# parlance/ctcdecode

Hardware: AMD Instinct MI355X
Metric: utterances/sec at B=256 T=1000 V=29 beam=100 (higher is better)
Workload: dtype f32; 1 GPU; BASELINE.json configs[1]: CTC prefix beam search, no LM, log-softmax of N(0,1) logits; HBM-resident tensors (input in HBM, the four result tensors left in HBM: `e2e`, with --full, is the host-to-host call); utterances_per_gpu=256, frames=1000, vocab=29, beam_width=100, cutoff_top_n=29, global_batch=256, ranks=1, devices_visible=1, parallelism=single GPU, threads_per_workgroup=default

## Files before the change

ctcdecode_amd/csrc/beam_core.h:

```cpp
#pragma once
#include <stddef.h>
#include <stdint.h>

#include "exact_math.h"
#include "exact_math_f64.h"
#include "lm_tables.h"
#include "stl_emul.h"
#if defined(CTC_ASSUME_CHECKED)
#include <cstdio>
#include <cstdlib>
#endif

#define CTC_RARE(x) __builtin_expect(!!(x), 0)
#if !defined(CTC_SPEC_UP)
#define CTC_SPEC_UP 1.5f
#endif
#if !defined(CTC_SPEC_DN)
#define CTC_SPEC_DN 0.7f
#endif
#if !defined(CTC_SPEC_OVER_SHIFT)
#define CTC_SPEC_OVER_SHIFT 2
#endif
#define CTC_USUAL(x) __builtin_expect(!!(x), 1)

// ... 189 lines not shown
  w.rev_lpc = carve_ptr<float>(deep ? q : p, K);
  w.cch = carve_ptr<int>(p, (size_t)d.Vc_max);
  w.clpbuf = carve_ptr<float>(p, 2 * (size_t)d.Vc_max); w.clp = w.clpbuf;
  w.rank_of = carve_ptr<int16_t>(p, d.use_rank_table ? (size_t)d.V : 0);
  w.skey = carve_ptr<uint32_t>(deep ? q : p, S);
  w.surv = carve_ptr<int>(p, 3 * K + 4);
  const size_t lcap = (d.K <= kSmallK && d.Vc_max <= kMidVc) ? (size_t)kHotCap + 64 : (size_t)kListCap + 4;
  w.bins = carve_ptr<int>(p, kBins + kBins / 16 + 4); w.list = carve_ptr<uint32_t>(p, lcap);
  w.lslot = carve_ptr<int>(p, lcap);
  w.hotge = carve_ptr<int>(p, lcap > (size_t)kListCap + 4 ? (size_t)kHotCap : 0);
#if defined(CTC_EXP_LCP_TABLE)
  w.lcpst = carve_ptr<int>(p, (lcap > (size_t)kListCap + 4 && !d.lm) ? (size_t)7 * kSmallK : 0);
#else
  w.lcpst = nullptr;
#endif
  w.bitmap = carve_ptr<uint32_t>(huge ? q : p, 2 * ((S + 63) / 64 + 17));
  w.wpre = huge ? carve_ptr<uint32_t>(q, (S + 63) / 64 + 2) : reinterpret_cast<uint32_t *>(w.bins);
  w.fin = carve_ptr<int>(BIG ? q : p, d.lm ? 2 * K : K);
  w.apos = carve_ptr<int>(BIG ? q : p, K);
  w.sstack = carve_ptr<int>(p, 3 * (2 * 32 + 2));
  w.vars = carve_ptr<int>(p, VAR_COUNT);
  w.sinfo = carve_ptr<uint32_t>(p, BIG ? K : S);
  w.pos = carve_ptr<uint32_t>(BIG ? q : p, K + 2);
  char *&rr = (BIG || FARREP) ? q : p;
  w.ek = carve_ptr<uint64_t>(rr, huge ? 2 * S : S); w.lr = carve_ptr<uint16_t>(rr, (2 * S + 2) * (huge ? 2 : 1));
  w.stage_skey = deep ? 0 : 1;
  if (far_bytes) *far_bytes = (size_t)(q - far);
  return (size_t)(p - base);
}

struct StreamState {
  int *hdr;
  int *arrays;
  int finish;
};
enum { SH_FRAMES = 0, SH_N, SH_POOL, SH_WLOG, SH_MAXKEY, SH_DANGER, SH_MINKEY,
       SH_SP_PRED, SH_SP_GAP, SH_SP_MARGIN,
       SH_WORDS = 12 };
constexpr int kStateArrays = 14;
constexpr int kStateArraysLm = kStateArrays + kBeamArraysLm;
CTC_HD int state_arrays(int lm) { return lm ? kStateArraysLm : kStateArrays; }

struct StepIn {
  int t;
  int Vc;
  int blank_rank;
  int identity;
  float blank_prob;
};


CTC_HD int div_p2(int v, int d) { return v >> __builtin_ctz((unsigned)d); }
CTC_HD int ceil_div_p2(int v, int d) { return div_p2(v + d - 1, d); }

CTC_HD double ctc_log_f64(double v) {
  return ctcmath::log_f64(v, ctcmath::tables64());
}

CTC_HD int ceil_log2_u32(uint32_t v) {
  return v <= 1u ? 0 : 32 - __builtin_clz(v - 1u);
}
CTC_HD int ceil_log2_u64(uint64_t v) {
  return v <= 1 ? 0 : 64 - __builtin_clzll(v - 1);
}

struct OutRefs {
  int32_t *tok, *ts;
  float *score;
  int32_t *len;
  int32_t *n_results;
  int K, T_stride;
  int32_t *c_hdr, *c_ent;
  uint32_t *c_rag;
  unsigned *c_count;
  unsigned c_cap;
  int32_t *m_hdr, *m_ent, *m_done;
  uint32_t *m_rag;
  unsigned m_cap;
};
enum : int { ST_COMPACT_OVERFLOW = 3, ST_INPUT_TIMEOUT = 4,
             ST_NEED_HOST = 5,
             ST_CB_DANGER = 6 };

struct SlotCtx {
  const Beam *pb;
  int n, Vnb, brank;
  uint64_t vmagic;
};

template <class X>
struct FullSyncView {
  X &x;
  CTC_HD int tid() const { return x.tid(); }
  CTC_HD int nt() const { return x.nt(); }
  CTC_HD void sync() { x.sync_full(); }
  CTC_HD int uni(int v) const { return x.uni(v); }
  CTC_HD void block_scan_u32(uint32_t mine, uint32_t *base_out, uint32_t *total_out) { x.block_scan_u32(mine, base_out, total_out); }
  CTC_HD int lanes() const { return x.lanes(); }
  CTC_HD auto ballot(bool p) const { return x.ballot(p); }
  template <class M> CTC_HD int count(M m) const { return x.count(m); }
  template <class M> CTC_HD int count_below(M m) const { return x.count_below(m); }
  CTC_HD uint32_t first_lane(uint32_t v) const { return x.first_lane(v); }
};

#if defined(CTC_ASSUME_CHECKED)
#define CTC_ASSUME(c) do { if (!(c)) { std::fprintf(stderr, "beam_core.h:%d: assumption violated: %s\n", __LINE__, #c); std::abort(); } } while (0)
#elif defined(__clang__)
#define CTC_ASSUME(c) __builtin_assume(c)
#else
#define CTC_ASSUME(c) do { if (!(c)) __builtin_unreachable(); } while (0)
#endif

template <class X, bool IDENT, int SMALLV = 0, bool LM = false, bool LAZY = false, bool FARREP = LAZY, bool HUGE = false, bool WORDLM = false, bool CB = false>
struct Decoder {
  using EO = EkOps<HUGE>;
  using Ek = typename EO::E;
  using LrT = typename EO::Pos;
  static constexpr int kClsK = SMALLV == 2 ? kMidK : kSmallK, kClsVc = SMALLV == 2 ? kMidVc : kSmallV, kClsSlots = kClsK * (2 + kClsVc);
  CTC_HD Ek *ekp() const { return reinterpret_cast<Ek *>(w.ek); }
  CTC_HD LrT *lrp() const { return reinterpret_cast<LrT *>(w.lr); }
  X &x;
  Work &w;
  const Dims d;
  const int blank;
  PoolNode *pool;
  int *pool_up;
  int *pool_thi;
  bool long_t = false;
  const int pool_cap;
  const uint64_t *tbl;
  const ctclm::LmView *lm;

  CTC_HD Decoder(X &x_, Work &w_, const Dims &d_, int blank_, PoolNode *pool_, int *pool_up_, int pool_cap_, const uint64_t *tbl_,
                 const ctclm::LmView *lm_ = nullptr)
      : x(x_), w(w_), d(d_), blank(blank_), pool(pool_), pool_up(pool_up_), pool_thi(pool_up_ + pool_cap_), pool_cap(pool_cap_), tbl(tbl_), lm(lm_) {
    if (LM) {
      const ctclm::DictNode root = lm->dict[0];
      root_lo = (int)root.mask_lo; root_hi = (int)root.mask_hi; root_fc = (int)root.first_child;
      lm_char_v = lm->char_based != 0; lm_wide_v = lm->dict_wide != 0; lm_space = lm->space_id;
      lm_alpha = lm->alpha; lm_beta = lm->beta;
      lm_dict = lm->dict;
    }
  }
  CTC_HD int node_tstep(const PoolNode &pn, int id) const { return (int)(pn.cht >> 16) | (CTC_RARE(long_t) ? pool_thi[id] << 16 : 0); }
  CTC_HD void set_node_time(int id, int ch, int tstep, float lpc) const {
    pool[id].lpc = lpc;
    pool[id].cht = PoolNode::pack(ch, tstep);
    if (CTC_RARE(long_t)) pool_thi[id] = tstep >> 16;
  }

  CTC_HD float lse(float a, float b) const { return ctcmath::lse(a, b, tbl); }

  static constexpr bool kRankEpoch = SMALLV == 2 && !IDENT && X::kRankEpoch;
  CTC_HD static int16_t rank_tag(int t, int r) { return (int16_t)(uint16_t)((((uint32_t)t & 1023u) << 6) | (uint32_t)r); }
  static constexpr bool kTailZero = IDENT && SMALLV && !LAZY && X::kZeroKeyTail;
  CTC_HD void zero_key_tail(int from) {
    if (!kTailZero) return;
    for (int i = from + x.tid(); i < kClsSlots; i += x.nt()) w.skey[i] = 0u;
  }

  static constexpr bool kSpec = SMALLV && (!LM || (X::kSpecLm && !CB)) && !LAZY && X::kSpecSelect;
#if defined(CTC_EXP_HOT_PRELIST)
  static constexpr bool kHotPre = LAZY && !LM && !SMALLV && !HUGE;
#else
  static constexpr bool kHotPre = false;
#endif
  struct HotPre { uint32_t thr; int cap; uint32_t *key; int *slot; };
  uint32_t st_gap = 0;
  uint32_t hot_anchor = 0;
  static constexpr bool kA1Overlap = kSpec && X::kA1Overlap;
// ... 1569 lines not shown
            } else {
              logp = child_logp(w.anc[j], c, lp);
              o_lpc = w.rev_lpc[j];
            }
            if (LM && lm_scores(c)) logp = lm_apply(logp, lm_window(b, child ? j : w.anc[j], c));
            o_b = CTC_NEG_MAX; o_nb = logp; o_sc = logp;
          }
          nb.bprev[k] = o_b; nb.nbprev[k] = o_nb; nb.score[k] = o_sc; nb.lpc[k] = o_lpc;
        }
        if (r_lm) lm_emit(b, (self || child) ? j : w.anc[j], self ? -1 : c, nb, k);
        if (r_prob) {
          const uint32_t ks = keys_in_ord ? (uint32_t)ord[k] : w.skey[s];
          kloc = ks > kloc ? ks : kloc;
          kmin = ks < kmin ? ks : kmin;
        }
      }
    }
    if (x.uni((int)r_prob_any)) {
      x.wave_max_to(&pv[P_NMAXKEY], kloc);
      if (LM) x.wave_min_to(&pv[P_NMINKEY], kmin);
    }
    if (CTC_RARE(last || exact || (N <= K && x.uni(w.vars[VAR_DANGER]) != 0))) {
      int *fin = fin_nxt();
      for (int q = tid; q < n_new; q += nt) {
        const int r = exact ? rk[q] : q;
        fin[q] = r;
        w.apos[r] = q;
      }
    } else if (lm_cb) {
      const int *fc = fin_cur();
      int *fn = fin_nxt();
      for (int q = tid; q < d.K; q += nt) fn[q] = fc[q];
    }
    if (!IDENT && !kRankEpoch) {
      x.sync();
      for (int r = tid; r < Vc; r += nt) w.rank_of[w.cch[r]] = -1;
    }
    if (stage && tid < d.V) w.clpbuf[((in.t + 1) & 1) * d.Vc_max + tid] = stage_val;
    if ((kSpec || kHotPre) && stage) x.row_max_store(&w.vars[VAR_ROWMAX], stage_val, d.V);
    x.mark(7);
    x.sync_full();
    x.mark(9);
    if (LM && CTC_RARE(lm_cb) && x.uni(w.vars[VAR_LMMISS]) != 0) return ST_NEED_HOST;
    if (kTailZero && LM) {
      const int S_next = n_new * (2 + Vnb);
      if (CTC_RARE(S_next < S))
        for (int i = S_next + tid; i < S; i += nt) w.skey[i] = 0u;
    }
    {
      if (!kSpec) {
        int wl = 32;
        st_gap = 0;
        if (N > K) {
          const uint32_t gap = st_maxkey > tau ? st_maxkey - tau : 0;
          wl = (gap ? 32 - __builtin_clz(gap) : 0) + 1;
          wl = wl < 10 ? 10 : (wl > 32 ? 32 : wl);
          st_gap = kHotPre ? (hot_anchor > tau ? hot_anchor - tau : 0u) : gap;
        }
        st_wlog = wl;
        st_maxkey = (uint32_t)x.uni(pv[P_NMAXKEY]);
      }
      if (LM) st_minkey = (uint32_t)x.uni(pv[P_NMINKEY]);
      st_n = n_new;
      st_pool = pool_count + n_new;
    }
    x.tick();
    x.dump(in.t, n_new, nb.node, nb.dep, nb.lcp, nb.score);
    x.mark(8);
    st_par ^= 1;
    return ST_OK;
  }

  template <class T, class C>
  CTC_HD void sort_like_std(T *v, int n, C before) {
    const int tid = x.tid(), nt = x.nt();
    constexpr int kTaskCap = (kBins + kBins / 16) / 6;
    if (n <= 16 || n / 17 + 1 > kTaskCap) {
      if (tid == 0) stlemu::sort(v, 0, n, before, w.sstack);
      x.sync();
      return;
    }
    stlemu::sort_parallel(x, v, n, before, w.bins, w.bins + 3 * kTaskCap, w.surv, w.vars + VAR_TAU);
  }

  CTC_HD int finish(bool had_steps, int max_depth, const OutRefs *outs, int item) {
    const OutRefs o = *x.fresh(outs);
    const int T_stride = o.T_stride;
    const size_t ko = (size_t)o.K * (size_t)o.T_stride;
    int32_t *out_tok = o.tok + (size_t)item * ko, *out_ts = o.ts + (size_t)item * ko;
    float *out_score = o.score + (size_t)item * o.K;
    int32_t *out_len = o.len + (size_t)item * o.K;
    int32_t *n_results = o.n_results ? o.n_results + item : nullptr;
    select_beams();
    const Beam &b = w.cur;
    const int tid = x.tid(), nt = x.nt();
    const int n = st_n;
    if (SMALLV) { CTC_ASSUME(n >= 1 && n <= kClsK); CTC_ASSUME(d.K <= kClsK); }
    const int nres = n < d.K ? n : d.K;
    if (!had_steps)
      for (int k = tid; k < nres; k += nt) fin_cur()[k] = k;
    x.sync();
    float *ext = w.sc_new;
    float *approx = w.b_new;
    {
      const float *sc = b.score;
      const int *ch = b.ch;
      uint64_t *pk = sort_scratch();
      if (LM) {
        for (int a = tid; a < n; a += nt) {
          if (CTC_RARE(lm_cb) && b.dfc[a] == kLmPending) continue;
          const bool partial = !lm_char_() && b.dep[a] > 0 && ch[a] != lm_space;
          const bool word_here = partial && lm_allows(b, a, lm_space);
          const double wcond = word_here ? mk_f64(b.spc_lo[a], b.spc_hi[a]) : ctclm::kOovScore;
          float e = sc[a];
          if (partial) {
            float score = 0.0f;
            score = (float)(wcond * lm_alpha);
            score = (float)((double)score + lm_beta);
            e += score;
          }
          ext[a] = e;
          double total = mk_f64(b.acc_lo[a], b.acc_hi[a]);
          uint32_t st = (uint32_t)b.lmst[a];
          int cl = b.lmcl[a];
          if (b.dep[a] == 0) {
            total += lm_cond_(&st, &cl, lm->w_bos);
          } else if (partial) {
            total += wcond;
            if (word_here) { st = (uint32_t)b.spst[a]; cl = b.spcl[a]; }
            else {
              st = (lm_cb && lm->clean0 == 0) ? lm->s0 : 0u;
              cl = 0;
            }
          }
          total += lm_cond_(&st, &cl, lm->w_eos);
          double ap = (double)e;
          ap = ap - (double)(size_t)b.dep[a] * lm_beta;
          ap -= total * lm_alpha;
          approx[a] = (float)ap;
        }
        x.sync();
        if (CTC_RARE(lm_cb) && x.uni(w.vars[VAR_LMMISS]) != 0) return ST_NEED_HOST;
      }
      for (int p = tid; p < nres; p += nt) {
        const int a = fin_cur()[p];
        pk[p] = (key48(ord_f32(LM ? ext[a] : sc[a]), mk_info(ch[a], 0, 0)) << 16) | (uint64_t)a;
      }
      x.sync();
      auto before = [](uint64_t a, uint64_t c) { return (a >> 16) > (c >> 16); };
      sort_like_std(pk, nres, before);
      if (LM) {
        for (int p = tid; p < nres; p += nt) {
          const int a = (int)(pk[p] & 0xFFFFu);
          pk[p] = (key48(ord_f32(sc[a]), mk_info(ch[a], 0, 0)) << 16) | (uint64_t)a;
        }
        x.sync();
      }
      sort_like_std(pk, nres, before);
      for (int p = tid; p < nres; p += nt) fin_cur()[p] = (int)(pk[p] & 0xFFFFu);
    }
    if (tid == 0 && n_results) *n_results = nres;
    x.sync();
    for (int p = tid; p < nres; p += nt) {
      const int j = fin_cur()[p];
      out_score[p] = LM ? -approx[j] : -b.score[j];
      out_len[p] = b.dep[j];
    }
    int *row_of = w.pinr, *owner = w.e;
    for (int p = tid; p < nres; p += nt) row_of[fin_cur()[p]] = p;
    for (int j = tid; j < nres; j += nt) {
      int o = j - 1;
      const int l = b.lcp[j];
      while (o >= 0 && b.lcp[o] >= l) --o;
      owner[j] = o;
    }
    x.sync();
    x.mark(4);
    const bool compact = o.c_hdr != nullptr;
    unsigned cbase = 0;
    uint32_t ctotal = 0;
    if (compact) {
      for (int j = tid; j < nres; j += nt) {
        const int lo = b.lcp[j] > 0 ? b.lcp[j] : 0;
        w.pos[j] = (uint32_t)(b.dep[j] > lo ? b.dep[j] - lo : 0);
      }
      if (tid == 0) w.pos[nres] = 0;
      x.sync();
      const uint32_t total = x.scan_excl(w.pos, nres + 1);
      if (tid == 0) w.vars[VAR_CUT] = (int)x.global_add(o.c_count, total);
      x.sync();
      cbase = (unsigned)x.uni(w.vars[VAR_CUT]);
      ctotal = total;
      const bool fits = cbase + total <= o.c_cap && cbase + total >= cbase;
      if (tid == 0) {
        int32_t *h = o.c_hdr + (size_t)item * 4;
        h[0] = fits ? nres : 0; h[1] = fits ? (int32_t)total : 0; h[2] = (int32_t)cbase; h[3] = 0;
        if (!fits) w.vars[VAR_STATUS] = ST_COMPACT_OVERFLOW;
      }
      if (!fits) return ST_COMPACT_OVERFLOW;
      for (int j = tid; j < nres; j += nt) {
        int32_t *e = o.c_ent + ((size_t)item * o.K + j) * 4;
        e[0] = row_of[j]; e[1] = b.lcp[j] > 0 ? b.lcp[j] : 0; e[2] = b.dep[j]; e[3] = (int32_t)(cbase + w.pos[j]);
      }
    }
    const int maxseg = max_depth / kExpress + 1;
    for (int idx = tid; idx < nres * maxseg; idx += nt) {
      const int i = idx / nres, j = idx - i * nres;
      const int dj = b.dep[j];
      const int lo = b.lcp[j] > 0 ? b.lcp[j] : 0;
      const int base = ((dj - 1) / kExpress) * kExpress;
      if (dj <= 0 || i > base / kExpress) continue;
      int dd = i == 0 ? dj : base - (i - 1) * kExpress;
      int stop = i == 0 ? base : dd - kExpress;
      if (dd <= lo) continue;
      stop = stop < lo ? lo : stop;
      int xn;
      if (i == 0) {
        xn = b.node[j];
      } else {
        xn = b.up[j];
        for (int h = 1; h < i; ++h) xn = pool_up[xn];
      }
      if (compact) {
        uint32_t *seg = o.c_rag + (size_t)cbase + w.pos[j] - lo;
        while (dd > stop) {
          const PoolNode pn = pool[xn];
          seg[dd - 1] = pn.cht;
          xn = pn.parent;
          --dd;
        }
        continue;
      }
      const size_t row = (size_t)row_of[j] * T_stride;
      int32_t *tk = out_tok + row, *ts = out_ts + row;
      while (dd > stop) {
        const PoolNode pn = pool[xn];
        tk[dd - 1] = pn.ch();
        ts[dd - 1] = node_tstep(pn, xn);
        xn = pn.parent;
        --dd;
      }
    }
    if (compact) {
      if (o.m_done) {
        x.sync_full();
        const bool mirror = cbase + ctotal <= o.m_cap;
        if (mirror) {
          for (uint32_t i = (uint32_t)tid; i < ctotal; i += (uint32_t)nt) o.m_rag[cbase + i] = o.c_rag[cbase + i];
          const int32_t *es = o.c_ent + (size_t)item * o.K * 4;
          int32_t *ed = o.m_ent + (size_t)item * o.K * 4;
          for (int i = tid; i < nres * 4; i += nt) ed[i] = es[i];
          if (tid < 4) o.m_hdr[(size_t)item * 4 + tid] = o.c_hdr[(size_t)item * 4 + tid];
        }
        x.fence_system();
        x.sync_full();
        if (tid == 0) x.store_system(&o.m_done[item], mirror ? 1 : 2);
      }
      return ST_OK;
    }
    x.sync_full();
    x.mark(15);
    const int grp = x.group(), ngr = x.ngroups(), lane = x.lane(), lanes = x.lanes();
    constexpr int kU = 8;
    for (int j = 1 + grp; j < nres; j += ngr) {
      const size_t row = (size_t)row_of[j] * T_stride;
      const int hi = b.lcp[j];
      const int o0 = owner[j];
      for (int q0 = lane; q0 < hi; q0 += lanes * kU) {
        int32_t tk[kU], ts[kU];
        for (int u = 0; u < kU; ++u) {
          const int q = q0 + u * lanes;
          if (q < hi) {
            int o = o0;
            while (b.lcp[o] > q) o = owner[o];
            const size_t src = (size_t)row_of[o] * T_stride + q;
            tk[u] = out_tok[src];
            ts[u] = out_ts[src];
          }
        }
        for (int u = 0; u < kU; ++u) {
          const int q = q0 + u * lanes;
          if (q < hi) { out_tok[row + q] = tk[u]; out_ts[row + q] = ts[u]; }
        }
      }
    }
    return ST_OK;
  }
};

struct PrunedRows {
  const int *cnt;
  const int *ch;
  const float *lp;
  int stride;
};

template <bool IDENT, int SMALLV = 0, bool LM = false, bool LAZY = false, bool FARREP = LAZY, bool HUGE = false, bool WORDLM = false, bool CB = false, class X>
CTC_HD int decode_utterance(X &x, Work &w, const Dims &d, int blank, const float *rows, const PrunedRows *pr, int len,
                            PoolNode *pool, int *pool_up, int pool_cap, const uint64_t *tbl, const OutRefs *outs, int item,
                            const StreamState *ss = nullptr, const ctclm::LmView *lm = nullptr, const float *raw = nullptr,
                            int raw_log = 1, const int *frames_ready = nullptr) {
  if (SMALLV == 1) { CTC_ASSUME(d.K >= 1 && d.K <= kSmallK); CTC_ASSUME(d.V >= 1 && d.V <= kSmallV); CTC_ASSUME(d.Vc_max >= 1 && d.Vc_max <= kSmallV); CTC_ASSUME(blank >= 0 && blank < kSmallV); }
  if (SMALLV == 2) { CTC_ASSUME(d.K >= 1 && d.K <= kMidK); CTC_ASSUME(d.V >= 1 && d.V <= kMidV); CTC_ASSUME(d.Vc_max >= 1 && d.Vc_max <= kMidVc); }
  using Dec0 = Decoder<X, IDENT, SMALLV, LM, LAZY, FARREP, HUGE, WORDLM, CB>;
  Dec0 dec(x, w, d, blank, pool, pool_up, pool_cap, tbl, lm);
  const int t0 = ss ? x.uni(ss->hdr[SH_FRAMES]) : 0;
  dec.long_t = (long long)t0 + len > 65536;
  if (t0 > 0) dec.load_state(*ss); else dec.init();
  dec.prime_a1(t0);
  const int tid = x.tid(), nt = x.nt();
  const int width = IDENT ? d.V : pr->stride;
  const bool prefetch = width <= nt;
  float pre_lp = 0.f;
  int pre_ch = 0, pre_cnt = 0;
  int ready_cached = 0;
  bool gave_up = false;
  auto wait_frames = [&](int need) {
    if (frames_ready != nullptr && need > ready_cached && !gave_up) {
      for (int spins = 0;; ++spins) {
        ready_cached = x.load_system(frames_ready);
        if (ready_cached >= need) break;
        if (spins > (1 << 20)) { w.vars[VAR_INTO] = 1; gave_up = true; break; }
        x.nap();
      }
    }
  };
  if (prefetch && len > 0) {
    if (!IDENT) {
      pre_cnt = pr->cnt[0];
      if (tid < width) { pre_ch = pr->ch[tid]; pre_lp = pr->lp[tid]; }
    } else if (tid < width) {
      wait_frames(1);
      pre_lp = rows[tid];
    }
  }
  if (IDENT && prefetch && len > 0) {
    if (tid < d.V) { w.clpbuf[(t0 & 1) * d.Vc_max + tid] = pre_lp; dec.note_lp(pre_lp); }
    if (Dec0::kSpec || Dec0::kHotPre) x.row_max_store(&w.vars[VAR_ROWMAX], pre_lp, d.V);
    x.sync();
  }
  for (int t = 0; t < len; ++t) {
    StepIn in;
    in.t = t0 + t;
    in.blank_prob = 0.f;
    if (LM) {
      const float rb = raw[(size_t)t * d.V + blank];
      in.blank_prob = raw_log ? rb : (float)ctc_log_f64((double)rb);
    }
    x.trace_frame(in.t);
    bool stage = false;
    int next_cnt = 0;
    float next_val = 0.f;
    using Dec = Dec0;
    if (IDENT) {
      in.Vc = d.V;
      in.identity = 1;
      in.blank_rank = blank;
      if (prefetch) {
        w.clp = w.clpbuf + ((t0 + t) & 1) * d.Vc_max;
        stage = t + 1 < len;
        if (stage && tid < d.V) {
          wait_frames(t + 2);
          pre_lp = rows[(size_t)(t + 1) * d.V + tid];
        }
        next_cnt = stage ? d.V : 0;
        next_val = pre_lp;
      } else {
// ... 85 lines not shown
```

ctcdecode_amd/csrc/ctcdecode_amd.hip:

```cpp
#include <hip/hip_runtime.h>

#include <cfloat>
#include <chrono>
#include <cmath>
#include <cstdio>
#include <cstring>
#include <algorithm>
#include <limits>
#include <atomic>
#include <condition_variable>
#include <functional>
#include <mutex>
#include <thread>
#include <string>
#include <vector>

#include "../../include/ctcdecode_amd.h"
#define CTC_EXACT_MATH_HOST_TABLES
#include "decode_kernel.h"
#include "exact_math_f64.h"
#include "lm_build.h"
#include "lm_callback.h"
#include "compact_results.h"
#include "stream_peek.h"
// ... 1535 lines not shown

static int launch_elementwise(ctcd_decoder *d, const float *in, float *out, size_t n, const int32_t *lens, int T, int V, hipStream_t stream, int dt,
                              bool to_log) {
  const int blocks = (int)std::min<size_t>((n + 255) / 256, 4096);
  const PrepassEntry *e = pp_pick(to_log ? CTCD_PP_PROB_TO_LOG : CTCD_PP_WIDEN, 0, dt, V);
  if (!e) return fail(CTCD_EINTERNAL, "no elementwise pre-pass for this input dtype");
  const void *fn = e->fn;
  void *args[] = {(void *)&in, (void *)&out, (void *)&n, (void *)&lens, (void *)&T, (void *)&V};
  HIP_TRY(hipLaunchKernel(fn, dim3(blocks), dim3(256), args, 0, stream));
  HIP_TRY(hipGetLastError());
  d->pre_fn[0] = fn;
  return CTCD_OK;
}

struct PruneFns { const void *rows, *wg, *wg_reg, *logits, *resolve; };
static PruneFns prune_fns(int dt, int V) {
  PruneFns f;
  f.rows = pp_pick(CTCD_PP_PRUNE_ROWS, 0, dt, V)->fn;
  f.wg = pp_pick(CTCD_PP_PRUNE_WG, 0, dt, V)->fn;
  const PrepassEntry *reg = pp_pick(CTCD_PP_PRUNE_WG, 1, dt, V);
  f.wg_reg = reg ? reg->fn : f.wg;
  f.logits = pp_pick(CTCD_PP_PRUNE_LOGITS, 0, dt, V)->fn;
  f.resolve = pp_pick(CTCD_PP_RESOLVE, 0, dt, V)->fn;
  return f;
}
}

int ctcd_debug_last_prepass(const ctcd_decoder *d, int32_t out[CTCD_PREPASS_FIELDS]) {
  if (!d || !out) return fail(CTCD_EINVAL, "decoder == NULL or out == NULL");
  for (int s = 0; s < 4; ++s) {
    int32_t *o = out + 4 * s;
    o[0] = o[1] = o[2] = o[3] = 0;
    if (!d->pre_fn[s]) continue;
    const PrepassEntry *e = pp_find(d->pre_fn[s]);
    if (!e) return fail(CTCD_EINTERNAL, "the last call launched a pre-pass kernel that is not in the table");
    o[0] = e->kernel; o[1] = e->a; o[2] = s == 3 ? (d->pre_resolve_global ? 1 : 0) : e->b; o[3] = e->dt;
  }
  return CTCD_OK;
}
int ctcd_debug_prepass_table(int32_t *out, int cap) {
  const int n = (int)(sizeof(kPrepass) / sizeof(kPrepass[0]));
  for (int i = 0; out && i < n && i < cap; ++i) {
    const PrepassEntry &e = kPrepass[i];
    int32_t *o = out + 5 * i;
    o[0] = e.kernel; o[1] = e.a; o[2] = e.b; o[3] = e.dt; o[4] = e.vmax;
  }
  return n;
}

static int decode_common(ctcd_decoder *d, const float *probs, const int32_t *seq_lens, int B, int T, int V, int beam,
                         double cutoff_prob, int cutoff_top_n, int blank_id, int log_input, int32_t *out_tok, int32_t *out_ts,
                         float *out_sc, int32_t *out_len, int32_t *n_results, void *stream_, const StreamCall *sc,
                         ctcd_scorer *scorer = nullptr, const CompactOut *co = nullptr, const int *frames_ready = nullptr) {
  if (!d) return fail(CTCD_EINVAL, "decoder == NULL");
  if (scorer && scorer->device != d->device) return fail(CTCD_EINVAL, "the scorer's tables live on another device than the decoder");
  if (scorer && (int)scorer->host.labels.size() != V) return fail(CTCD_EINVAL, "the scorer was built for a different number of labels");
  const int out_T = sc ? sc->out_T : T;
  const bool no_rows = (sc && out_T == 0) || co;
  if (co && (out_T > 65536 || V > 65535)) return fail(CTCD_EUNSUPPORTED, "compact results pack label and frame into 16 bits each");
  int rc = check_args(B, T, V, beam, cutoff_top_n, blank_id, probs, no_rows ? (const void *)d : (const void *)out_tok,
                      no_rows ? (const void *)d : (const void *)out_ts, out_sc, out_len);
  if (rc) return rc;
  std::lock_guard<std::mutex> lock(d->mu);
  hipStream_t stream = (hipStream_t)stream_;
  CTC_ON_DEVICE(d->device);
  if (B == 0) {
    if (!sc) d->last_order_items = 0;
    return CTCD_OK;
  }
  cutoff_prob = used_cutoff_prob(cutoff_prob);
  const Dims dims = make_dims(beam, V, cutoff_top_n, cutoff_prob, scorer != nullptr);
  const ScorerKind sk = !scorer ? kNoScorer : scorer->cbl ? kCallbackScorer
                        : (!scorer->host.char_based && !scorer->host.dict_wide && !d->general_lm_kernel) ? kWordScorer : kGeneralScorer;
  const LaunchSwitches sw{d->no_fixed_layout, d->profile, d->tl_armed, d->cu_sharing, d->subtree_mode, d->subtree_on};
  const LaunchPlan plan = plan_launch(dims, B, d->threads, d->max_lds, d->cu_count, sw, sk, frames_ready != nullptr,
                                      [](const KernelKey &k) { return kernel_entry(k) != nullptr; });
  if (plan.rc) return fail(plan.rc, plan.msg);
  const KernelEntry *kernel = kernel_entry(plan.key);
  const int threads = plan.threads;
  size_t lds = plan.lds;
  const size_t far_bytes = plan.far_bytes;
  if ((rc = d->far.ensure((size_t)B * far_bytes))) return rc;

  const size_t kt = co ? 0 : (size_t)B * beam * out_T;
  if (co && !(sc && sc->no_clear)) {
    HIP_TRY(hipMemsetAsync(co->count, 0, 4, stream));
    HIP_TRY(hipMemsetAsync(co->hdr, 0, (size_t)B * 16, stream));
  }
  if (kt && !(sc && sc->no_clear)) {
    HIP_TRY(hipMemsetAsync(out_tok, 0, kt * 4, stream));
    HIP_TRY(hipMemsetAsync(out_ts, 0, kt * 4, stream));
  }
  if ((!sc || sc->any_eos) && !(sc && sc->no_clear)) {
    HIP_TRY(hipMemsetAsync(out_sc, 0, (size_t)B * beam * 4, stream));
    HIP_TRY(hipMemsetAsync(out_len, 0, (size_t)B * beam * 4, stream));
    if (sc && n_results) HIP_TRY(hipMemsetAsync(n_results, 0, (size_t)B * 4, stream));
  }

  if (!d->tables_ready) {
    if ((rc = d->tables.ensure(sizeof(ctcmath::Tables)))) return rc;
    HIP_TRY(hipMemcpy(d->tables.p, ctcmath::host_tables().w, sizeof(ctcmath::Tables), hipMemcpyHostToDevice));
    d->tables_ready = true;
  }
  char **st_base = nullptr;
  int *st_cap = nullptr;
  unsigned char *st_eos = nullptr;
  if (sc) {
    const size_t off_cap = (size_t)B * 8, off_len = off_cap + (size_t)B * 4, off_eos = off_len + (size_t)B * 4, need = (off_eos + (size_t)B + 31) & ~(size_t)15;
    if ((rc = d->st_args.ensure(2 * need))) return rc;
    if (d->h_stargs_cap < need) {
      for (int i = 0; i < 2; ++i) {
        if (d->ev_stargs[i]) HIP_TRY(hipEventSynchronize(d->ev_stargs[i]));
        if (d->h_stargs[i]) (void)hipHostFree(d->h_stargs[i]);
        d->h_stargs[i] = nullptr;
        HIP_TRY(hipHostMalloc((void **)&d->h_stargs[i], need, hipHostMallocDefault));
        if (!d->ev_stargs[i]) HIP_TRY(hipEventCreateWithFlags(&d->ev_stargs[i], hipEventDisableTiming));
      }
      d->h_stargs_cap = need;
    }
    const int slot = (int)(d->stream_calls++ & 1);
    HIP_TRY(hipEventSynchronize(d->ev_stargs[slot]));
    char *hb = d->h_stargs[slot];
    for (int b = 0; b < B; ++b) {
      ctcd_stream *st = sc->states[b];
      ((char **)hb)[b] = st->block;
      ((int *)(hb + off_cap))[b] = (int)(st->cap_frames * beam + 1);
      ((int *)(hb + off_len))[b] = sc->lens[b];
      hb[off_eos + b] = sc->is_eos[b] ? 1 : 0;
    }
    char *db = (char *)d->st_args.p + (size_t)slot * need;
    HIP_TRY(hipMemcpyAsync(db, hb, off_eos + (size_t)B, hipMemcpyHostToDevice, stream));
    HIP_TRY(hipEventRecord(d->ev_stargs[slot], stream));
    st_base = (char **)db;
    st_cap = (int *)(db + off_cap);
    st_eos = (unsigned char *)db + off_eos;
    seq_lens = (const int32_t *)(db + off_len);
  }
  std::fill(d->pre_fn, d->pre_fn + 4, nullptr);
  const int32_t *pre_lens = (sc && sc->row_lens) ? sc->row_lens : seq_lens;
  int dt = d->in_dtype;
  d->last_in_dtype = dt;
  if (dt != CTCD_DTYPE_F32 && scorer && log_input != 2 && T > 0) {
    if ((rc = d->lsm.ensure((size_t)B * T * V * 4))) return rc;
    if (pre_lens) HIP_TRY(hipMemsetAsync(d->lsm.p, 0, (size_t)B * T * V * 4, stream));
    if ((rc = launch_elementwise(d, probs, (float *)d->lsm.p, (size_t)B * T * V, pre_lens, T, V, stream, dt, false))) return rc;
    probs = (const float *)d->lsm.p;
    dt = CTCD_DTYPE_F32;
  }

  const bool fuse_logits = log_input == 2 && dims.use_rank_table && T > 0 && !scorer && !d->no_fused_logits && V % 4 == 0 && V > 256 &&
                           V <= 16384 && std::min(cutoff_top_n, V) <= 64 && ((uintptr_t)probs & (4 * in_elem_bytes(dt) - 1)) == 0;
  if (log_input == 2 && !fuse_logits) {
    if (T > 0) {
      if ((rc = d->lsm.ensure((size_t)B * T * V * 4))) return rc;
      if (pre_lens) HIP_TRY(hipMemsetAsync(d->lsm.p, 0, (size_t)B * T * V * 4, stream));
      if ((rc = launch_log_softmax(d, probs, (float *)d->lsm.p, (long long)B * T, pre_lens, T, V, stream, dt))) return rc;
      probs = (const float *)d->lsm.p;
      dt = CTCD_DTYPE_F32;
    }
    log_input = 1;
  }
  const long long pool_stride = (long long)beam * T + 1;
  if (!sc && (rc = d->pool.ensure((size_t)B * pool_stride * (sizeof(PoolNode) + 2 * sizeof(int))))) return rc;
  if ((rc = d->status.ensure((size_t)B * 8))) return rc;
  HIP_TRY(hipMemsetAsync(d->status.p, 0xff, (size_t)B * 4, stream));
  d->last_stream = stream;
  const float *logp = probs;
  d->prune_flagged_rows = 0;
  d->flagged_pending = false;
  if (dims.use_rank_table && T > 0) {
    const long long rows = (long long)B * T;
    const int stride = dims.Vc_max;

    if ((rc = d->pr_cnt.ensure((size_t)rows * 4))) return rc;
    if ((rc = d->pr_ch.ensure((size_t)rows * stride * 4))) return rc;
    if ((rc = d->pr_lp.ensure((size_t)rows * stride * 4))) return rc;
// ... 1560 lines not shown
```

ctcdecode_amd/csrc/decode_kernel.h:

```cpp
#pragma once
#include <hip/hip_runtime.h>

#include <cstddef>
#include <cstdint>

#include "beam_core.h"
#include "launch_plan.h"

namespace ctcdk {

using namespace ctcbeam;

#define CTC_BALLOT(p) __builtin_amdgcn_ballot_w64(p)
#define CTC_DPP(old, v, ctrl, rowmask) __builtin_amdgcn_update_dpp((int)(old), (int)(v), (ctrl), (rowmask), 0xf, false)

template <class Op>
__device__ __forceinline__ int wave_scan(int v, const int ident, Op op) {
  v = op(CTC_DPP(ident, v, 0x111, 0xf), v);
  v = op(CTC_DPP(ident, v, 0x112, 0xf), v);
  v = op(CTC_DPP(ident, v, 0x114, 0xf), v);
  v = op(CTC_DPP(ident, v, 0x118, 0xf), v);
  v = op(CTC_DPP(ident, v, 0x142, 0xa), v);
  v = op(CTC_DPP(ident, v, 0x143, 0xc), v);
  return v;
// ... 761 lines not shown
  if (PROF == 1) x.last = (long long)wall_clock64();
  const size_t f0 = a.frame_off ? (size_t)__builtin_amdgcn_readfirstlane(a.frame_off[b]) : 0;
  PrunedRows prow;
  if (PRUNED) {
    prow.cnt = a.pr_cnt + (size_t)b * a.T + f0;
    prow.ch = a.pr_ch + ((size_t)b * a.T + f0) * a.pr_stride;
    prow.lp = a.pr_lp + ((size_t)b * a.T + f0) * a.pr_stride;
    prow.stride = a.pr_stride;
  }
  PoolNode *pool = a.pool + (size_t)b * a.pool_stride;
  int *pool_up = a.pool_up + (size_t)b * 2 * a.pool_stride;
  int pool_cap = (int)a.pool_stride;
  StreamState ss;
  if (a.st_base) {
    char *base = a.st_base[b];
    ss.hdr = (int *)base;
    ss.arrays = ss.hdr + SH_WORDS;
    ss.finish = a.st_eos[b];
    pool = (PoolNode *)(base + a.st_pool_off);
    pool_cap = a.st_poolcap[b];
    pool_up = (int *)(pool + pool_cap);
  }
#if defined(__HIP_DEVICE_COMPILE__)
  const OutRefs *outs = (const OutRefs *)((const char *)__builtin_amdgcn_kernarg_segment_ptr() + offsetof(KernelArgs, outs));
#else
  const OutRefs *outs = &a.outs;
#endif
  const ctclm::LmView *lmv = nullptr;
#if defined(__HIP_DEVICE_COMPILE__)
  if (LM) lmv = (const ctclm::LmView *)((const char *)__builtin_amdgcn_kernarg_segment_ptr() + offsetof(KernelArgs, lm));
#else
  if (LM) lmv = &a.lm;
#endif
  int st;
  if (LM == 3) {
    __shared__ unsigned cb_n;
    size_t fo = f0;
    unsigned log_pos = 0, q_total = 0;
    for (;;) {
      const int before = a.st_base ? __builtin_amdgcn_readfirstlane(__hip_atomic_load(&ss.hdr[SH_FRAMES], __ATOMIC_RELAXED, __HIP_MEMORY_SCOPE_AGENT)) : 0;
      if (PRUNED) {
        prow.cnt = a.pr_cnt + (size_t)b * a.T + fo;
        prow.ch = a.pr_ch + ((size_t)b * a.T + fo) * a.pr_stride;
        prow.lp = a.pr_lp + ((size_t)b * a.T + fo) * a.pr_stride;
      }
      st = decode_utterance<!PRUNED, (LAYOUT == 3 ? 0 : LAYOUT), true, BIG != 0, BIG != 0 || OCC2, BIG == 3, false, true>(x, w, a.dims, a.blank, PRUNED ? nullptr : a.probs + ((size_t)b * a.T + fo) * a.V,
                                  PRUNED ? &prow : (const PrunedRows *)nullptr, len, pool, pool_up, pool_cap, tbl, outs, b,
                                  a.st_base ? &ss : (const StreamState *)nullptr, lmv, a.raw + ((size_t)b * a.T + fo) * a.V, a.raw_log, (const int *)nullptr);
      if (st != ctcbeam::ST_NEED_HOST || a.cb_log_len == nullptr || !a.st_base) break;
      __threadfence_system();
      __syncthreads();
      const unsigned asked = (unsigned)w.vars[ctcbeam::VAR_LMQ];
      if (asked == 0) break;
      q_total += asked;
      if (threadIdx.x == 0) {
        unsigned n = 0;
        for (int spins = 0;; ++spins) {
          const unsigned ans = __hip_atomic_load(&a.cb_ans[b], __ATOMIC_ACQUIRE, __HIP_MEMORY_SCOPE_SYSTEM);
          n = __hip_atomic_load(a.cb_log_len, __ATOMIC_ACQUIRE, __HIP_MEMORY_SCOPE_SYSTEM);
          if (n == 0xFFFFFFFFu || ans >= q_total) break;
          if (spins > (1 << 21)) { n = 0xFFFFFFFFu; break; }
          __builtin_amdgcn_s_sleep(8);
        }
        cb_n = n;
      }
      __syncthreads();
      const unsigned n = cb_n;
      if (n == 0xFFFFFFFFu || n < log_pos) break;
      ctclm::NgSlot *ng = const_cast<ctclm::NgSlot *>(a.lm.ng);
      for (unsigned i = log_pos + threadIdx.x; i < n; i += blockDim.x) ng[a.cb_log_idx[i]] = a.cb_log_slot[i];
      log_pos = n;
      __threadfence();
      const int consumed = __builtin_amdgcn_readfirstlane(__hip_atomic_load(&ss.hdr[SH_FRAMES], __ATOMIC_RELAXED, __HIP_MEMORY_SCOPE_AGENT)) - before;
      __syncthreads();
      fo += (size_t)consumed;
      len -= consumed;
    }
  } else {
  st = decode_utterance<!PRUNED, (LAYOUT == 3 ? 0 : LAYOUT), LM != 0, BIG != 0, BIG != 0 || OCC2, BIG == 3, LM == 2, LM == 3>(x, w, a.dims, a.blank, PRUNED ? nullptr : a.probs + ((size_t)b * a.T + f0) * a.V,
                                  PRUNED ? &prow : (const PrunedRows *)nullptr, len, pool, pool_up, pool_cap, tbl, outs, b,
                                  a.st_base ? &ss : (const StreamState *)nullptr, lmv, LM ? a.raw + ((size_t)b * a.T + f0) * a.V : nullptr, a.raw_log,
                                  (PRUNED || kNoStreamedInput) ? (const int *)nullptr : a.frames_ready);
  }
  if (threadIdx.x == 0) {
    if (a.shape) a.shape[b] = 16 * w.vars[ctcbeam::VAR_QSTAT];
    a.status[b] = st;
    if (a.frames_done && a.st_base) a.frames_done[b] = ss.hdr[SH_FRAMES];
    if (LM == 3 && a.cb_done) {
      __threadfence_system();
      __hip_atomic_store(&a.cb_done[b], 1 + st, __ATOMIC_RELEASE, __HIP_MEMORY_SCOPE_SYSTEM);
    }
  }
  if (PROF == 2 && a.tl && b == 0) {
    __syncthreads();
    for (int i = threadIdx.x; i < 16 * kTlCap; i += blockDim.x) a.tl[i] = tlbuf[i];
  }
  if (PROF == 1 && threadIdx.x < 16) a.prof[(size_t)b * 16 + threadIdx.x] = prof[threadIdx.x];
}

#define CTC_KERNEL_GROUPS 12
#if defined(CTC_QUICK_BUILD) && CTC_QUICK_BUILD == 2
#define CTC_KERNEL_LIST(X) X(0, 0, 1, false, 1024, 2, false, 0) X(2, 0, 1, false, 1024, 2, false, 1) X(0, 0, 1, false, 1024, true, false, 1) X(2, 0, 1, false, 1024, true, false, 0) X(4, 0, 1, false, 1024, 2, false, 1)
#elif defined(CTC_QUICK_BUILD) && CTC_QUICK_BUILD == 3
#define CTC_KERNEL_LIST(X) X(0, 0, 1, false, CTC_QUICK_NT, false, false, 0)
#elif defined(CTC_QUICK_BUILD) && CTC_QUICK_BUILD == 4
#define CTC_KERNEL_LIST(X) X(0, 0, 2, true, 1024, false, false, 0) X(0, 0, 1, true, 1024, false, false, 1) X(0, 0, 0, true, 0, false, false, 1) X(0, 0, 0, false, 0, false, false, 0)
#elif defined(CTC_QUICK_BUILD)
#define CTC_KERNEL_LIST(X) \
  X(0, 0, 1, false, 1024, false, false, 0) X(2, 0, 1, false, 1024, false, false, 1) X(0, 0, 1, false, 1024, false, true, 1) X(4, 0, 1, false, 1024, false, false, 1) X(4, 0, 1, false, 1024, false, true, 0)
#else
#define CTC_KERNEL_LIST(X)                                                                                                          \
  X(0, 0, 1, false, 1024, false, false, 0) X(0, 0, 1, true, 1024, false, false, 1) X(2, 0, 1, false, 1024, false, false, 2)               \
  X(0, 1, 0, false, 0, false, false, 3) X(0, 1, 0, true, 0, false, false, 4) X(0, 2, 0, false, 0, false, false, 5) X(0, 2, 0, true, 0, false, false, 5) \
  X(0, 0, 0, false, 0, false, false, 6) X(0, 0, 0, true, 0, false, false, 6) X(0, 0, 1, false, 0, false, false, 7) X(0, 0, 1, true, 0, false, false, 7) \
  X(1, 1, 0, false, 0, false, false, 8) X(1, 1, 0, true, 0, false, false, 8) X(1, 0, 1, false, 0, false, false, 9) X(1, 0, 1, true, 0, false, false, 9) \
  X(1, 0, 0, false, 0, false, false, 10) X(1, 0, 0, true, 0, false, false, 10) X(0, 1, 3, false, 1024, false, false, 10)                                                       \
  X(0, 0, 0, false, 0, true, false, 11) X(0, 0, 0, true, 0, true, false, 11) X(0, 0, 1, false, 1024, true, false, 2)                     \
  X(0, 0, 1, true, 1024, true, false, 3) X(2, 0, 1, false, 1024, true, false, 4)                                                       \
  X(0, 0, 1, false, 1024, 2, false, 0) X(0, 0, 1, true, 1024, 2, false, 1) X(0, 0, 1, false, 1024, 2, true, 2) X(0, 0, 1, true, 1024, 2, true, 3) X(2, 0, 1, false, 1024, 2, false, 5) \
  X(0, 0, 1, false, 1024, false, true, 0) X(0, 0, 1, true, 1024, false, true, 1) X(0, 0, 1, false, 1024, true, true, 10) X(0, 0, 1, true, 1024, true, true, 11) \
  X(0, 1, 0, false, 0, true, false, 6) X(0, 1, 0, true, 0, true, false, 7) X(0, 2, 0, false, 0, true, false, 8) X(0, 2, 0, true, 0, true, false, 9) \
  X(0, 3, 0, false, 0, false, false, 5) X(0, 3, 0, true, 0, false, false, 4) X(0, 3, 0, false, 0, true, false, 6) X(0, 3, 0, true, 0, true, false, 7) \
  X(0, 1, 0, false, 1024, false, false, 9) X(0, 1, 0, true, 1024, false, false, 10) X(2, 1, 0, false, 1024, false, false, 11) \
  X(4, 0, 1, false, 1024, false, false, 3) X(5, 0, 1, false, 1024, false, false, 5) X(4, 0, 1, false, 1024, 2, false, 7) X(4, 0, 1, false, 1024, false, true, 9) \
  X(0, 0, 2, true, 1024, false, false, 0) \
  X(3, 0, 1, false, 1024, false, false, 1) X(3, 0, 1, true, 1024, false, false, 2) X(0, 0, 1, false, 1024, 3, false, 8) X(0, 0, 1, true, 1024, 3, false, 9) X(0, 0, 0, false, 0, 3, false, 10) X(0, 0, 0, true, 0, 3, false, 4) \
  X(0, 1, 0, false, 0, 3, false, 6) X(0, 1, 0, true, 0, 3, false, 7) X(0, 2, 0, false, 0, 3, false, 8) X(0, 2, 0, true, 0, 3, false, 9) X(0, 3, 0, false, 0, 3, false, 11) X(0, 3, 0, true, 0, 3, false, 5)
#endif

}
```

Baseline: 52240 utterances/s.

## Move output zeroing into decode kernel and stage tokens for vectorized row writes

Drops the host-side memsets of the token, timestep, score and length buffers for the non-streaming path. Each workgroup now writes full padded rows itself, zero-filling past each beam's depth and clearing unused beams and failed items. When the decoded tokens fit in LDS scratch, traceback is staged there and whole rows are written with int4 stores. The final sorts also run on one wave while the other waves do traceback. This removes a large separate memset pass over B*beam*T outputs, at the cost of more kernel code and more paths to keep correct.

```diff
diff --git a/ctcdecode_amd/csrc/beam_core.h b/ctcdecode_amd/csrc/beam_core.h
--- a/ctcdecode_amd/csrc/beam_core.h
+++ b/ctcdecode_amd/csrc/beam_core.h
@@ -295,10 +295,43 @@
              ST_NEED_HOST = 5,
              ST_CB_DANGER = 6 };
 
+CTC_HD void fill_zero(int32_t *p, size_t n, int me, int cnt) {
+  size_t head = (size_t)((0u - (unsigned)(reinterpret_cast<uintptr_t>(p) >> 2)) & 3u);
+  head = head < n ? head : n;
+  const size_t nv = (n - head) >> 2, done = head + 4 * nv;
+  for (size_t i = (size_t)me; i < head; i += (size_t)cnt) p[i] = 0;
+  Int4v *v = reinterpret_cast<Int4v *>(p + head);
+  for (size_t i = (size_t)me; i < nv; i += (size_t)cnt) v[i] = Int4v{0, 0, 0, 0};
+  for (size_t i = done + (size_t)me; i < n; i += (size_t)cnt) p[i] = 0;
+}
+template <class X>
+CTC_HD void clear_results(X &x, const OutRefs &o, int item, int first = 0) {
+  const int tid = x.tid(), nt = x.nt();
+  if (first >= o.K) return;
+  const size_t rows = (size_t)(o.K - first), at = (size_t)item * (size_t)o.K + (size_t)first;
+  if (o.tok) fill_zero(o.tok + at * (size_t)o.T_stride, rows * (size_t)o.T_stride, tid, nt);
+  if (o.ts) fill_zero(o.ts + at * (size_t)o.T_stride, rows * (size_t)o.T_stride, tid, nt);
+  for (size_t p = (size_t)tid; p < rows; p += (size_t)nt) { o.score[at + p] = 0.0f; o.len[at + p] = 0; }
+}
+template <class X>
+CTC_HD void clear_results_if_unfinished(X &x, const OutRefs &o, int item, int st) {
+  if (st == ST_POOL_OVERFLOW || st == ST_BAD_CONFIG || st == ST_INPUT_TIMEOUT) clear_results(x, o, item);
+}
+
 struct SlotCtx {
   const Beam *pb;
   int n, Vnb, brank;
   uint64_t vmagic;
+};
+
+template <class X>
+struct WaveView {
+  X &x;
+  CTC_HD int tid() const { return x.lane(); }
+  CTC_HD int nt() const { return x.lanes(); }
+  CTC_HD void sync() { x.wave_lds_fence(); }
+  CTC_HD int uni(int v) const { return x.uni(v); }
+  CTC_HD int atomic_add(int *p, int v) { return x.atomic_add(p, v); }
 };
 
 template <class X>
@@ -2034,6 +2067,28 @@
     }
     stlemu::sort_parallel(x, v, n, before, w.bins, w.bins + 3 * kTaskCap, w.surv, w.vars + VAR_TAU);
   }
+  template <class P, class T, class C>
+  CTC_HD void sort_like_std_on(P &xp, T *v, int n, C before) {
+    constexpr int kTaskCap = (kBins + kBins / 16) / 6;
+    if (n <= 16 || n / 17 + 1 > kTaskCap) {
+      if (xp.tid() == 0) stlemu::sort(v, 0, n, before, w.sstack);
+      xp.sync();
+      return;
+    }
+    stlemu::sort_parallel(xp, v, n, before, w.bins, w.bins + 3 * kTaskCap, w.surv, w.vars + VAR_TAU);
+  }
+  CTC_HD uint32_t *stage_area(uint32_t *cap) const {
+    const uint32_t K = (uint32_t)d.K, S = (uint32_t)d.S_max();
+    uint32_t *p = nullptr;
+    uint32_t c = 0;
+    if (!FARREP) { p = reinterpret_cast<uint32_t *>(w.ek + K); c = 3 * S - 2 * K; }
+    else if (w.stage_skey) { p = w.skey + 2 * K; c = S > 2 * K ? S - 2 * K : 0; }
+#if defined(CTC_STAGE_CAP_MAX)
+    c = c < (uint32_t)(CTC_STAGE_CAP_MAX) ? c : (uint32_t)(CTC_STAGE_CAP_MAX);
+#endif
+    *cap = c;
+    return p;
+  }
 
   CTC_HD int finish(bool had_steps, int max_depth, const OutRefs *outs, int item) {
     const OutRefs o = *x.fresh(outs);
@@ -2054,99 +2109,157 @@
     x.sync();
     float *ext = w.sc_new;
     float *approx = w.b_new;
-    {
-      const float *sc = b.score;
-      const int *ch = b.ch;
-      uint64_t *pk = sort_scratch();
+    const float *sc = b.score;
+    const int *ch = b.ch;
+    uint64_t *pk = sort_scratch();
+    if (LM) {
+      for (int a = tid; a < n; a += nt) {
+        if (CTC_RARE(lm_cb) && b.dfc[a] == kLmPending) continue;
+        const bool partial = !lm_char_() && b.dep[a] > 0 && ch[a] != lm_space;
+        const bool word_here = partial && lm_allows(b, a, lm_space);
+        const double wcond = word_here ? mk_f64(b.spc_lo[a], b.spc_hi[a]) : ctclm::kOovScore;
+        float e = sc[a];
+        if (partial) {
+          float score = 0.0f;
+          score = (float)(wcond * lm_alpha);
+          score = (float)((double)score + lm_beta);
+          e += score;
+        }
+        ext[a] = e;
+        double total = mk_f64(b.acc_lo[a], b.acc_hi[a]);
+        uint32_t st = (uint32_t)b.lmst[a];
+        int cl = b.lmcl[a];
+        if (b.dep[a] == 0) {
+          total += lm_cond_(&st, &cl, lm->w_bos);
+        } else if (partial) {
+          total += wcond;
+          if (word_here) { st = (uint32_t)b.spst[a]; cl = b.spcl[a]; }
+          else {
+            st = (lm_cb && lm->clean0 == 0) ? lm->s0 : 0u;
+            cl = 0;
+          }
+        }
+        total += lm_cond_(&st, &cl, lm->w_eos);
+        double ap = (double)e;
+        ap = ap - (double)(size_t)b.dep[a] * lm_beta;
+        ap -= total * lm_alpha;
+        approx[a] = (float)ap;
+      }
+      x.sync();
+      if (CTC_RARE(lm_cb) && x.uni(w.vars[VAR_LMMISS]) != 0) return ST_NEED_HOST;
+    }
+    for (int p = tid; p < nres; p += nt) {
+      const int a = fin_cur()[p];
+      pk[p] = (key48(ord_f32(LM ? ext[a] : sc[a]), mk_info(ch[a], 0, 0)) << 16) | (uint64_t)a;
+    }
+    int *row_of = w.pinr, *owner = w.e;
+    for (int j = tid; j < nres; j += nt) {
+      int o = j - 1;
+      const int l = b.lcp[j];
+      while (o >= 0 && b.lcp[o] >= l) --o;
+      owner[j] = o;
+      const int lo = l > 0 ? l : 0;
+      w.pos[j] = (uint32_t)(b.dep[j] > lo ? b.dep[j] - lo : 0);
+    }
+    if (tid == 0) w.pos[nres] = 0;
+    x.sync();
+    const uint32_t ctotal = x.scan_excl(w.pos, nres + 1);
+    const bool compact = o.c_hdr != nullptr;
+    unsigned cbase = 0;
+    bool fits = false;
+    if (compact) {
+      if (tid == 0) w.vars[VAR_CUT] = (int)x.global_add(o.c_count, ctotal);
+      x.sync();
+      cbase = (unsigned)x.uni(w.vars[VAR_CUT]);
+      fits = cbase + ctotal <= o.c_cap && cbase + ctotal >= cbase;
+    }
+    uint32_t stage_cap = 0;
+    uint32_t *stage = stage_area(&stage_cap);
+    const bool staged = !compact && !long_t && ctotal <= stage_cap;
+    uint32_t *seg = compact ? (fits ? o.c_rag + (size_t)cbase : nullptr) : (staged ? stage : nullptr);
+    const int maxseg = max_depth / kExpress + 1;
+    auto read_back = [&](int t0, int step) {
+      for (int idx = t0; idx < nres * maxseg; idx += step) {
+        const int i = idx / nres, j = idx - i * nres;
+        const int dj = b.dep[j];
+        const int lo = b.lcp[j] > 0 ? b.lcp[j] : 0;
+        const int base = ((dj - 1) / kExpress) * kExpress;
+        if (dj <= 0 || i > base / kExpress) continue;
+        int dd = i == 0 ? dj : base - (i - 1) * kExpress;
+        int stop = i == 0 ? base : dd - kExpress;
+        if (dd <= lo) continue;
+        stop = stop < lo ? lo : stop;
+        int xn;
+        if (i == 0) {
+          xn = b.node[j];
+        } else {
+          xn = b.up[j];
+          for (int h = 1; h < i; ++h) xn = pool_up[xn];
+        }
+        if (seg) {
+          uint32_t *sg = seg + w.pos[j] - lo;
+          while (dd > stop) {
+            const PoolNode pn = pool[xn];
+            sg[dd - 1] = pn.cht;
+            xn = pn.parent;
+            --dd;
+          }
+          continue;
+        }
+        const size_t row = (size_t)row_of[j] * T_stride;
+        int32_t *tk = out_tok + row, *ts = out_ts + row;
+        while (dd > stop) {
+          const PoolNode pn = pool[xn];
+          tk[dd - 1] = pn.ch();
+          ts[dd - 1] = node_tstep(pn, xn);
+          xn = pn.parent;
+          --dd;
+        }
+      }
+    };
+    auto before = [](uint64_t a, uint64_t c) { return (a >> 16) > (c >> 16); };
+    auto sorts = [&](auto &xp) {
+      const int t = xp.tid(), m = xp.nt();
+      sort_like_std_on(xp, pk, nres, before);
       if (LM) {
-        for (int a = tid; a < n; a += nt) {
-          if (CTC_RARE(lm_cb) && b.dfc[a] == kLmPending) continue;
-          const bool partial = !lm_char_() && b.dep[a] > 0 && ch[a] != lm_space;
-          const bool word_here = partial && lm_allows(b, a, lm_space);
-          const double wcond = word_here ? mk_f64(b.spc_lo[a], b.spc_hi[a]) : ctclm::kOovScore;
-          float e = sc[a];
-          if (partial) {
-            float score = 0.0f;
-            score = (float)(wcond * lm_alpha);
-            score = (float)((double)score + lm_beta);
-            e += score;
-          }
-          ext[a] = e;
-          double total = mk_f64(b.acc_lo[a], b.acc_hi[a]);
-          uint32_t st = (uint32_t)b.lmst[a];
-          int cl = b.lmcl[a];
-          if (b.dep[a] == 0) {
-            total += lm_cond_(&st, &cl, lm->w_bos);
-          } else if (partial) {
-            total += wcond;
-            if (word_here) { st = (uint32_t)b.spst[a]; cl = b.spcl[a]; }
-            else {
-              st = (lm_cb && lm->clean0 == 0) ? lm->s0 : 0u;
-              cl = 0;
-            }
-          }
-          total += lm_cond_(&st, &cl, lm->w_eos);
-          double ap = (double)e;
-          ap = ap - (double)(size_t)b.dep[a] * lm_beta;
-          ap -= total * lm_alpha;
-          approx[a] = (float)ap;
-        }
-        x.sync();
-        if (CTC_RARE(lm_cb) && x.uni(w.vars[VAR_LMMISS]) != 0) return ST_NEED_HOST;
-      }
-      for (int p = tid; p < nres; p += nt) {
-        const int a = fin_cur()[p];
-        pk[p] = (key48(ord_f32(LM ? ext[a] : sc[a]), mk_info(ch[a], 0, 0)) << 16) | (uint64_t)a;
-      }
-      x.sync();
-      auto before = [](uint64_t a, uint64_t c) { return (a >> 16) > (c >> 16); };
-      sort_like_std(pk, nres, before);
-      if (LM) {
-        for (int p = tid; p < nres; p += nt) {
+        for (int p = t; p < nres; p += m) {
           const int a = (int)(pk[p] & 0xFFFFu);
           pk[p] = (key48(ord_f32(sc[a]), mk_info(ch[a], 0, 0)) << 16) | (uint64_t)a;
         }
-        x.sync();
-      }
-      sort_like_std(pk, nres, before);
-      for (int p = tid; p < nres; p += nt) fin_cur()[p] = (int)(pk[p] & 0xFFFFu);
-    }
+        xp.sync();
+      }
+      sort_like_std_on(xp, pk, nres, before);
+    };
+    const bool pk_near = !FARREP || w.stage_skey != 0;
+    const bool split = seg != nullptr && pk_near && x.ngroups() > 1 && nres / 17 + 1 <= x.lanes();
+    if (split) {
+      if (x.group() == 0) {
+        WaveView<X> xw{x};
+        sorts(xw);
+      } else {
+        read_back(tid - x.lanes(), nt - x.lanes());
+      }
+      x.sync();
+    } else {
+      sorts(x);
+      if (seg) read_back(tid, nt);
+    }
+    for (int p = tid; p < nres; p += nt) fin_cur()[p] = (int)(pk[p] & 0xFFFFu);
     if (tid == 0 && n_results) *n_results = nres;
     x.sync();
     for (int p = tid; p < nres; p += nt) {
       const int j = fin_cur()[p];
       out_score[p] = LM ? -approx[j] : -b.score[j];
       out_len[p] = b.dep[j];
-    }
-    int *row_of = w.pinr, *owner = w.e;
-    for (int p = tid; p < nres; p += nt) row_of[fin_cur()[p]] = p;
-    for (int j = tid; j < nres; j += nt) {
-      int o = j - 1;
-      const int l = b.lcp[j];
-      while (o >= 0 && b.lcp[o] >= l) --o;
-      owner[j] = o;
-    }
+      row_of[j] = p;
+    }
+    clear_results(x, o, item, nres);
     x.sync();
     x.mark(4);
-    const bool compact = o.c_hdr != nullptr;
-    unsigned cbase = 0;
-    uint32_t ctotal = 0;
     if (compact) {
-      for (int j = tid; j < nres; j += nt) {
-        const int lo = b.lcp[j] > 0 ? b.lcp[j] : 0;
-        w.pos[j] = (uint32_t)(b.dep[j] > lo ? b.dep[j] - lo : 0);
-      }
-      if (tid == 0) w.pos[nres] = 0;
-      x.sync();
-      const uint32_t total = x.scan_excl(w.pos, nres + 1);
-      if (tid == 0) w.vars[VAR_CUT] = (int)x.global_add(o.c_count, total);
-      x.sync();
-      cbase = (unsigned)x.uni(w.vars[VAR_CUT]);
-      ctotal = total;
-      const bool fits = cbase + total <= o.c_cap && cbase + total >= cbase;
       if (tid == 0) {
         int32_t *h = o.c_hdr + (size_t)item * 4;
-        h[0] = fits ? nres : 0; h[1] = fits ? (int32_t)total : 0; h[2] = (int32_t)cbase; h[3] = 0;
+        h[0] = fits ? nres : 0; h[1] = fits ? (int32_t)ctotal : 0; h[2] = (int32_t)cbase; h[3] = 0;
         if (!fits) w.vars[VAR_STATUS] = ST_COMPACT_OVERFLOW;
       }
       if (!fits) return ST_COMPACT_OVERFLOW;
@@ -2154,46 +2267,6 @@
         int32_t *e = o.c_ent + ((size_t)item * o.K + j) * 4;
         e[0] = row_of[j]; e[1] = b.lcp[j] > 0 ? b.lcp[j] : 0; e[2] = b.dep[j]; e[3] = (int32_t)(cbase + w.pos[j]);
       }
-    }
-    const int maxseg = max_depth / kExpress + 1;
-    for (int idx = tid; idx < nres * maxseg; idx += nt) {
-      const int i = idx / nres, j = idx - i * nres;
-      const int dj = b.dep[j];
-      const int lo = b.lcp[j] > 0 ? b.lcp[j] : 0;
-      const int base = ((dj - 1) / kExpress) * kExpress;
-      if (dj <= 0 || i > base / kExpress) continue;
-      int dd = i == 0 ? dj : base - (i - 1) * kExpress;
-      int stop = i == 0 ? base : dd - kExpress;
-      if (dd <= lo) continue;
-      stop = stop < lo ? lo : stop;
-      int xn;
-      if (i == 0) {
-        xn = b.node[j];
-      } else {
-        xn = b.up[j];
-        for (int h = 1; h < i; ++h) xn = pool_up[xn];
-      }
-      if (compact) {
-        uint32_t *seg = o.c_rag + (size_t)cbase + w.pos[j] - lo;
-        while (dd > stop) {
-          const PoolNode pn = pool[xn];
-          seg[dd - 1] = pn.cht;
-          xn = pn.parent;
-          --dd;
-        }
-        continue;
-      }
-      const size_t row = (size_t)row_of[j] * T_stride;
-      int32_t *tk = out_tok + row, *ts = out_ts + row;
-      while (dd > stop) {
-        const PoolNode pn = pool[xn];
-        tk[dd - 1] = pn.ch();
-        ts[dd - 1] = node_tstep(pn, xn);
-        xn = pn.parent;
-        --dd;
-      }
-    }
-    if (compact) {
       if (o.m_done) {
         x.sync_full();
         const bool mirror = cbase + ctotal <= o.m_cap;
@@ -2210,9 +2283,50 @@
       }
       return ST_OK;
     }
+    const int grp = x.group(), ngr = x.ngroups(), lane = x.lane(), lanes = x.lanes();
+    if (staged) {
+      for (int j = grp; j < nres; j += ngr) {
+        const size_t row = (size_t)row_of[j] * T_stride;
+        int32_t *tk = out_tok + row, *ts = out_ts + row;
+        const int dj = b.dep[j] < T_stride ? b.dep[j] : T_stride;
+        const int lo = b.lcp[j] > 0 ? b.lcp[j] : 0;
+        const int o0 = owner[j];
+        auto word = [&](int q) -> uint32_t {
+          int e = j;
+          if (q < lo) {
+            e = o0;
+            while (b.lcp[e] > q) e = owner[e];
+          }
+          const int l = b.lcp[e] > 0 ? b.lcp[e] : 0;
+          return stage[w.pos[e] + (uint32_t)(q - l)];
+        };
+        const unsigned mis_tk = (unsigned)(reinterpret_cast<uintptr_t>(tk) >> 2) & 3u, mis_ts = (unsigned)(reinterpret_cast<uintptr_t>(ts) >> 2) & 3u;
+        int head = mis_tk == mis_ts ? (int)((4u - mis_tk) & 3u) : T_stride;
+        head = head < T_stride ? head : T_stride;
+        const int nv = (T_stride - head) >> 2;
+        for (int q = lane; q < head; q += lanes) {
+          const uint32_t v = q < dj ? word(q) : 0u;
+          tk[q] = (int32_t)(v & 0xFFFFu); ts[q] = (int32_t)(v >> 16);
+        }
+        Int4v *tk4 = reinterpret_cast<Int4v *>(tk + head), *ts4 = reinterpret_cast<Int4v *>(ts + head);
+        for (int v4 = lane; v4 < nv; v4 += lanes) {
+          const int q0 = head + 4 * v4;
+          uint32_t v[4];
+          for (int u = 0; u < 4; ++u) v[u] = q0 + u < dj ? word(q0 + u) : 0u;
+          tk4[v4] = Int4v{(int)(v[0] & 0xFFFFu), (int)(v[1] & 0xFFFFu), (int)(v[2] & 0xFFFFu), (int)(v[3] & 0xFFFFu)};
+          ts4[v4] = Int4v{(int)(v[0] >> 16), (int)(v[1] >> 16), (int)(v[2] >> 16), (int)(v[3] >> 16)};
+        }
+        for (int q = head + 4 * nv + lane; q < T_stride; q += lanes) {
+          const uint32_t v = q < dj ? word(q) : 0u;
+          tk[q] = (int32_t)(v & 0xFFFFu); ts[q] = (int32_t)(v >> 16);
+        }
+      }
+      x.mark(15);
+      return ST_OK;
+    }
+    read_back(tid, nt);
     x.sync_full();
     x.mark(15);
-    const int grp = x.group(), ngr = x.ngroups(), lane = x.lane(), lanes = x.lanes();
     constexpr int kU = 8;
     for (int j = 1 + grp; j < nres; j += ngr) {
       const size_t row = (size_t)row_of[j] * T_stride;
@@ -2235,6 +2349,13 @@
           if (q < hi) { out_tok[row + q] = tk[u]; out_ts[row + q] = ts[u]; }
         }
       }
+    }
+    for (int j = grp; j < nres; j += ngr) {
+      const int dj = b.dep[j];
+      if (dj >= T_stride) continue;
+      const size_t at = (size_t)row_of[j] * T_stride + (size_t)dj;
+      fill_zero(out_tok + at, (size_t)(T_stride - dj), lane, lanes);
+      fill_zero(out_ts + at, (size_t)(T_stride - dj), lane, lanes);
     }
     return ST_OK;
   }
diff --git a/ctcdecode_amd/csrc/ctcdecode_amd.hip b/ctcdecode_amd/csrc/ctcdecode_amd.hip
--- a/ctcdecode_amd/csrc/ctcdecode_amd.hip
+++ b/ctcdecode_amd/csrc/ctcdecode_amd.hip
@@ -1641,16 +1641,17 @@
   const size_t far_bytes = plan.far_bytes;
   if ((rc = d->far.ensure((size_t)B * far_bytes))) return rc;
 
+  const bool host_clears = sc || sk == kCallbackScorer;
   const size_t kt = co ? 0 : (size_t)B * beam * out_T;
   if (co && !(sc && sc->no_clear)) {
     HIP_TRY(hipMemsetAsync(co->count, 0, 4, stream));
     HIP_TRY(hipMemsetAsync(co->hdr, 0, (size_t)B * 16, stream));
   }
-  if (kt && !(sc && sc->no_clear)) {
+  if (kt && host_clears && !(sc && sc->no_clear)) {
     HIP_TRY(hipMemsetAsync(out_tok, 0, kt * 4, stream));
     HIP_TRY(hipMemsetAsync(out_ts, 0, kt * 4, stream));
   }
-  if ((!sc || sc->any_eos) && !(sc && sc->no_clear)) {
+  if (host_clears && (!sc || sc->any_eos) && !(sc && sc->no_clear)) {
     HIP_TRY(hipMemsetAsync(out_sc, 0, (size_t)B * beam * 4, stream));
     HIP_TRY(hipMemsetAsync(out_len, 0, (size_t)B * beam * 4, stream));
     if (sc && n_results) HIP_TRY(hipMemsetAsync(n_results, 0, (size_t)B * 4, stream));
diff --git a/ctcdecode_amd/csrc/decode_kernel.h b/ctcdecode_amd/csrc/decode_kernel.h
--- a/ctcdecode_amd/csrc/decode_kernel.h
+++ b/ctcdecode_amd/csrc/decode_kernel.h
@@ -867,6 +867,7 @@
                                   a.st_base ? &ss : (const StreamState *)nullptr, lmv, LM ? a.raw + ((size_t)b * a.T + f0) * a.V : nullptr, a.raw_log,
                                   (PRUNED || kNoStreamedInput) ? (const int *)nullptr : a.frames_ready);
   }
+  if (st != ctcbeam::ST_OK && !a.st_base) ctcbeam::clear_results_if_unfinished(x, *outs, b, st);
   if (threadIdx.x == 0) {
     if (a.shape) a.shape[b] = 16 * w.vars[ctcbeam::VAR_QSTAT];
     a.status[b] = st;
```

Result: no change. 52180 utterances/s (-0.1%).
